# hip-satomi/microbeSEG

Measured on AMD Instinct MI355X. Metric: training crops/sec (256px), higher is better.
Workload: dtype f32; 1 GPU; BASELINE configs[1]: DU-Net distance-map training step, filters [64, 1024], 256x256 crops, per-GPU batch 32, fp32, relu/bn, SmoothL1x2 + Adam(amsgrad); global_batch=32, parallelism=dp1, launch=eager

## Files before the change

include/mseg_hip.h:

```cpp
#ifndef MSEG_HIP_H
#define MSEG_HIP_H

#include <stddef.h>
#include <stdint.h>

#ifdef __cplusplus
extern "C" {
#endif

#define MSEG_OK 0
#define MSEG_EINVAL (-1)
#define MSEG_ELAUNCH (-2)
#define MSEG_EWORKSPACE (-3)

#define MSEG_ACT_NONE 0
#define MSEG_ACT_RELU 1
#define MSEG_ACT_LEAKY 2
#define MSEG_ACT_ELU 3
#define MSEG_ACT_MISH 4

#define MSEG_NORM_BN 0
#define MSEG_NORM_GN 1
#define MSEG_NORM_IN 2

// ... 35 lines not shown
  float* stats;
  int32_t stats_act;
  int32_t reserved0;
} MsegIgemm;

int mseg_igemm(const MsegIgemm* p, void* stream);

typedef struct MsegKernelInfo {
  char name[120];
  int32_t precision;
  int32_t launches;
  uint32_t grid, block;
  size_t workspace;
  int32_t stats_rows;
  int32_t reserved0;
} MsegKernelInfo;
int mseg_igemm_query(const MsegIgemm* p, MsegKernelInfo* info);
const char* mseg_last_kernel(void);
int mseg_f32_to_bf16(const float* src, uint16_t* dst, size_t n, void* stream);
size_t mseg_igemm_workspace_bytes(const MsegIgemm* p);
int mseg_igemm_set_persistent(int on);
int mseg_igemm_set_wide_tiles(int on);
int mseg_igemm_set_p8(int mode);

typedef struct MsegWgrad {
  MsegSrc P;
  MsegSrc Q[2];
  float* ws;
  float* dst;
  int32_t nq, Nch, Nch_store;
  int32_t NB, Hp, Wp, Hq, Wq;
  int32_t KH, KW, stride, pad;
  int32_t splits;
  int32_t phase;
  int32_t precision;
  int32_t reserved;
} MsegWgrad;

size_t mseg_wgrad_workspace_bytes(const MsegWgrad* p);
int mseg_wgrad(const MsegWgrad* p, void* stream);
int mseg_wgrad_query(const MsegWgrad* p, MsegKernelInfo* info);

int mseg_first_conv_fwd(const float* x4, const float* w, const float* bias, int N, int H, int W, int Cin, int Cout,
                        void* z, int z_dtype, void* stream);
#define MSEG_PIX_U8 0
#define MSEG_PIX_U16 1
// ... 167 lines not shown
```

microbeseg_amd/_lib.py:

```python
import ctypes as C
import os
import pathlib

_HERE = pathlib.Path(__file__).resolve().parent
LIB_PATH = _HERE / "libmseg_hip.so"

ACT = {"none": 0, "relu": 1, "leakyrelu": 2, "elu": 3, "mish": 4}
NORM = {"bn": 0, "gn": 1, "in": 2}
MODE_CONV, MODE_TCONV = 0, 1
EPI_PLAIN, EPI_SCATTER2X2 = 0, 1
MORDER_LINEAR, MORDER_PARITY = 0, 1
ST_F32, ST_BF16 = 0, 1


class MsegLibraryError(RuntimeError):
    pass


class MsegSrc(C.Structure):
    _fields_ = [("ptr", C.c_void_p), ("scale", C.c_void_p), ("shift", C.c_void_p),
                ("C", C.c_int32), ("act", C.c_int32), ("ss", C.c_int32), ("dtype", C.c_int32)]


class MsegIgemm(C.Structure):
# ... 29 lines not shown
                ("first_block", C.c_uint32), ("reserved", C.c_uint32)]


class MsegRangerJob(C.Structure):
    _fields_ = [("p", C.c_void_p), ("g", C.c_void_p), ("m", C.c_void_p), ("v", C.c_void_p), ("slow", C.c_void_p),
                ("n", C.c_uint64), ("rows", C.c_int32), ("step_lr", C.c_float), ("flags", C.c_uint32),
                ("reserved", C.c_uint32)]


_P = C.c_void_p
_I = C.c_int
_F = C.c_float
_D = C.c_double
_SZ = C.c_size_t

SIGNATURES = {
    "mseg_igemm": (_I, [C.POINTER(MsegIgemm), _P]),
    "mseg_igemm_workspace_bytes": (_SZ, [C.POINTER(MsegIgemm)]),
    "mseg_igemm_query": (_I, [C.POINTER(MsegIgemm), C.POINTER(MsegKernelInfo)]),
    "mseg_last_kernel": (C.c_char_p, []),
    "mseg_igemm_set_persistent": (_I, [_I]),
    "mseg_igemm_set_wide_tiles": (_I, [_I]),
    "mseg_igemm_set_p8": (_I, [_I]),
    "mseg_f32_to_bf16": (_I, [_P, _P, _SZ, _P]),
    "mseg_first_conv_fwd": (_I, [_P, _P, _P, _I, _I, _I, _I, _I, _P, _I, _P]),
    "mseg_frame_minmax": (_I, [_P, _I, _SZ, _P, _P]),
    "mseg_first_conv_fwd_raw": (_I, [_P, _I, _I, _I, _I, _I, _P, _P, _P, _I, _P, _I, _P]),
    "mseg_frame_normalize": (_I, [_P, _I, _I, _I, _I, _I, _P, _P, _P]),
    "mseg_first_wgrad_workspace_bytes": (_SZ, [_I, _I, _I, _I]),
    "mseg_first_wgrad": (_I, [_P, _P, _I, _I, _I, _I, _I, _P, _P, _P]),
    "mseg_wgrad_workspace_bytes": (_SZ, [C.POINTER(MsegWgrad)]),
    "mseg_wgrad": (_I, [C.POINTER(MsegWgrad), _P]),
    "mseg_wgrad_query": (_I, [C.POINTER(MsegWgrad), C.POINTER(MsegKernelInfo)]),
    "mseg_pack_weight": (_I, [_P, _P, _I, _I, _I, _I, _I, _I, _I, _I, _P]),
    "mseg_pack_job_blocks": (C.c_uint, [_I, _I, _I]),
    "mseg_pack_weights_multi": (_I, [_P, _I, C.c_uint, _P]),
    "mseg_norm_workspace_bytes": (_SZ, [_I, _I, _I]),
    "mseg_norm_set_tails": (_I, [_I]),
    "mseg_norm_set_finish": (_I, [_I]),
    "mseg_norm_stats_from_conv": (_I, [_P, _I, _I, C.c_longlong, _P, _P, _F, _P, _P, _P, _P, _P, _P, _F, _P, _P]),
    "mseg_norm_stats": (_I, [_P, _I, _I, _I, _I, _I, _I, _P, _P, _F, _P, _P, _P, _P, _P, _P, _F, _P, _P, _P]),
    "mseg_activation": (_I, [_P, _I, _I, _I, _I, _I, _P, _P]),
    "mseg_bn_eval_coeffs": (_I, [_P, _P, _P, _P, _F, _I, _P, _P, _P]),
    "mseg_norm_bwd": (_I, [_P, _P, _I, _I, _I, _I, _I, _I, _P, _P, _P, _P, _P, _P, _P, _P, _P, _P]),
    "mseg_maxpool2x2_fwd": (_I, [C.POINTER(MsegSrc), _I, _I, _I, _P, _P]),
    "mseg_maxpool2x2_bwd": (_I, [C.POINTER(MsegSrc), _I, _I, _I, _P, _P, _I, _P]),
# ... 95 lines not shown
```

microbeseg_amd/csrc/igemm.hip:

```cpp
#include "common.h"
#include "igemm_common.h"
#include "bf16_affine.h"

int igemm_p8_try(const MsegIgemm& p, int tr, int m_fastest, int cus, hipStream_t st);

__device__ float g_ident_scale[MSEG_MAX_CH];
__device__ float g_ident_shift[MSEG_MAX_CH];
__global__ void init_ident_kernel() {
  for (int i = blockIdx.x * blockDim.x + threadIdx.x; i < MSEG_MAX_CH; i += gridDim.x * blockDim.x) {
    g_ident_scale[i] = 1.f;
    g_ident_shift[i] = 0.f;
  }
}


template <int BM, int BN, bool PER_SAMPLE, bool GENERIC_ACT>
__global__ __launch_bounds__(256) void igemm_kernel(const MsegIgemm p) {
  using Cfg = IgemmCfg<BM, BN>;
  constexpr int STAGE = (BM + BN) * LDS_STRIDE;
  __shared__ __attribute__((aligned(16))) float lds[2 * STAGE + 4];
  unsigned* tapmask_s = reinterpret_cast<unsigned*>(lds + 2 * STAGE);

  const int tid = threadIdx.x;
  const int lane = tid & 63;
  const int wave = tid >> 6;
  const int wm = wave / Cfg::WN, wn = wave % Cfg::WN;

// ... 186 lines not shown
    }
    float* An = lds + (cur ^ 1) * STAGE;
#ifdef MSEG_ABLATE
    STAMP(s2);
    if (!(abl & 8)) commit(An, An + BM * LDS_STRIDE);
    STAMP(s3);
    if (!(abl & 2)) __syncthreads();
    STAMP(s4);
    t_issue += s1 - s0; t_mfma += s2 - s1; t_commit += s3 - s2; t_bar += s4 - s3;
#else
    commit(An, An + BM * LDS_STRIDE);
    __syncthreads();
#endif
    cur ^= 1;
    have = have_next;
  }

#ifdef MSEG_ABLATE
  if ((abl & 32) && p.dst1 && lane == 0 && blockIdx.x < 1024) {
    float* dbg = p.dst1 + ((size_t)blockIdx.x * 4 + wave) * 4;
    dbg[0] = (float)t_issue; dbg[1] = (float)t_mfma; dbg[2] = (float)t_commit; dbg[3] = (float)t_bar;
  }
#endif
  igemm_epilogue<IgemmCfg<BM, BN>>(acc, m0, n0, wm, wn, lane, M);
}

template <int BM, int BN, int TR, bool PER_SAMPLE, bool SB = false>
__global__ __launch_bounds__(256) void igemm_fast_kernel(const MsegIgemm p) {
  using Cfg = IgemmCfg<BM, BN>;
  constexpr int STAGE = (BM + BN) * LDS_STRIDE;
  __shared__ __attribute__((aligned(16))) float lds[(SB ? 1 : 2) * STAGE];

  const int tid = threadIdx.x;
  const int lane = tid & 63;
  const int wave = tid >> 6;
  const int wm = wave / Cfg::WN, wn = wave % Cfg::WN;
  const int M = p.NB * p.Ho * p.Wo;
  const int ntiles_n = (p.Ngemm + BN - 1) / BN;
  const int lid = (int)xcd_logical_id(blockIdx.x, gridDim.x);
  const int tile_m = lid / ntiles_n;
  const int tile_n = lid - tile_m * ntiles_n;
  const int m0 = tile_m * BM, n0 = tile_n * BN;
  const int T = p.KH * p.KW;
  const int srow = tid >> 3, scol = tid & 7;

  const TapGeom geom = make_geom(p);
  const long long tile_px = tile_base_pixel(p, geom, m0, M);
  int pix0[Cfg::AROWS];
  int rown[Cfg::AROWS];
  unsigned vmask[Cfg::AROWS];
#pragma unroll
  for (int i = 0; i < Cfg::AROWS; ++i) {
    const RowInfo r = decode_row(p, m0 + srow + 32 * i, M);
    const int iy0 = (r.oy * geom.sm - geom.dir * geom.pad) >> geom.sh, ix0 = (r.ox * geom.sm - geom.dir * geom.pad) >> geom.sh;
    pix0[i] = (int)(((long long)r.n * p.Hi + iy0) * p.Wi + ix0 - tile_px);
    rown[i] = r.n < 0 ? 0 : r.n;
    unsigned mk = 0u;
    for (int t = 0; t < T; ++t) {
      const int ky = t / p.KW, kx = t - ky * p.KW;
      int iy, ix;
      mk |= (unsigned)tap_coord(geom, r, ky, kx, iy, ix) << t;
    }
    vmask[i] = mk;
  }

  f32x16 acc[Cfg::MB][Cfg::NB];
#pragma unroll
  for (int a = 0; a < Cfg::MB; ++a)
#pragma unroll
    for (int b = 0; b < Cfg::NB; ++b)
#pragma unroll
      for (int r = 0; r < 16; ++r) acc[a][b][r] = 0.f;

  const int nchunks = (p.Cin + KC - 1) / KC;
  const int C0 = p.src[0].C;
  const unsigned OOB = 0x80000000u;

  const __amdgpu_buffer_rsrc_t rs0 = __builtin_amdgcn_make_buffer_rsrc(
      const_cast<float*>(p.src[0].ptr + tile_px * p.src[0].C), 0, 0x7ffffff0, 0x00020000);
  const __amdgpu_buffer_rsrc_t rs1 = __builtin_amdgcn_make_buffer_rsrc(
      const_cast<float*>((p.nsrc > 1 ? p.src[1].ptr : p.src[0].ptr) + tile_px * (p.nsrc > 1 ? p.src[1].C : p.src[0].C)), 0,
      0x7ffffff0, 0x00020000);
  const __amdgpu_buffer_rsrc_t rsw = __builtin_amdgcn_make_buffer_rsrc(const_cast<float*>(p.w), 0,
                                                                        T * p.Npad * p.Kpad * 4, 0x00020000);
  unsigned wvoff[Cfg::BROWS];
#pragma unroll
  for (int i = 0; i < Cfg::BROWS; ++i) wvoff[i] = ((unsigned)(n0 + srow + 32 * i) * (unsigned)p.Kpad + scol * 4u) * 4u;

  constexpr int NSC = (TR == 0) ? 1 : (PER_SAMPLE ? Cfg::AROWS : 1);
  float4 ra[Cfg::AROWS], rb[Cfg::BROWS], rsc[NSC], rsh[NSC];
  float rm[Cfg::AROWS];
  unsigned rowoff[Cfg::AROWS];
  int ract = 0;
  int cur_chunk = -1;
  bool cur_s1 = false;

  auto issue = [&](int chunk, int t, int ky, int kx) {
    const int c = chunk * KC + scol * 4;
    if (chunk != cur_chunk) {
      cur_chunk = chunk;
      cur_s1 = (p.nsrc > 1) && (chunk * KC >= C0);
      const unsigned sC4 = (unsigned)(cur_s1 ? p.src[1].C : p.src[0].C) * 4u;
      const unsigned cl4 = (unsigned)(cur_s1 ? c - C0 : c) * 4u;
#pragma unroll
      for (int i = 0; i < Cfg::AROWS; ++i) rowoff[i] = (unsigned)pix0[i] * sC4 + cl4;
      if (TR != 0) {
        const MsegSrc& s = cur_s1 ? p.src[1] : p.src[0];
        ract = s.act;
        const bool has_aff = s.scale != nullptr;
        const float* scp = has_aff ? s.scale : g_ident_scale;
        const float* shp = has_aff ? s.shift : g_ident_shift;
        const unsigned cl = (c < p.Cin) ? (cl4 >> 2) : 0u;
#pragma unroll
        for (int i = 0; i < NSC; ++i) {
          const size_t o = (size_t)(PER_SAMPLE ? rown[i] : 0) * (has_aff ? (unsigned)s.ss : 0u) + cl;
          rsc[i] = *reinterpret_cast<const float4*>(scp + o);
          rsh[i] = *reinterpret_cast<const float4*>(shp + o);
        }
      }
    }
    const unsigned cbit = (c < p.Cin) ? (1u << t) : 0u;
    const unsigned sC4 = (unsigned)(cur_s1 ? p.src[1].C : p.src[0].C) * 4u;
    const unsigned delta = (unsigned)(geom.dir * ((ky >> geom.sh) * p.Wi + (kx >> geom.sh))) * sC4;
#pragma unroll
    for (int i = 0; i < Cfg::AROWS; ++i) {
      const bool ok = (vmask[i] & cbit) != 0u;
      const unsigned vo = ok ? rowoff[i] + delta : OOB;
      const f32x4 v = cur_s1 ? __builtin_bit_cast(f32x4, __builtin_amdgcn_raw_buffer_load_b128(rs1, vo, 0, 0))
                             : __builtin_bit_cast(f32x4, __builtin_amdgcn_raw_buffer_load_b128(rs0, vo, 0, 0));
      ra[i] = make_float4(v[0], v[1], v[2], v[3]);
      if (TR != 0) rm[i] = ok ? 1.f : 0.f;
    }
    const unsigned wso = ((unsigned)t * (unsigned)p.Npad * (unsigned)p.Kpad + (unsigned)chunk * KC) * 4u;
#pragma unroll
    for (int i = 0; i < Cfg::BROWS; ++i) {
      const f32x4 v = __builtin_bit_cast(f32x4, __builtin_amdgcn_raw_buffer_load_b128(rsw, wvoff[i], wso, 0));
      rb[i] = make_float4(v[0], v[1], v[2], v[3]);
    }
  };

  auto commit = [&](float* As, float* Bs) {
    const float lo = (ract == MSEG_ACT_RELU) ? 0.f : -3.402823466e38f;
#pragma unroll
    for (int i = 0; i < Cfg::AROWS; ++i) {
      float4 v = ra[i];
      if (TR != 0) {
        if (TR == 2) {
          v = act_fwd4(v, ract);
        } else {
          v.x = clamp_lo(v.x, lo); v.y = clamp_lo(v.y, lo); v.z = clamp_lo(v.z, lo); v.w = clamp_lo(v.w, lo);
        }
        const float4 sc = rsc[PER_SAMPLE ? i : 0], sh = rsh[PER_SAMPLE ? i : 0];
        const float m = rm[i];
        v.x = (v.x * sc.x + sh.x) * m; v.y = (v.y * sc.y + sh.y) * m;
        v.z = (v.z * sc.z + sh.z) * m; v.w = (v.w * sc.w + sh.w) * m;
      }
      *reinterpret_cast<float4*>(As + (srow + 32 * i) * LDS_STRIDE + scol * 4) = v;
    }
#pragma unroll
    for (int i = 0; i < Cfg::BROWS; ++i)
      *reinterpret_cast<float4*>(Bs + (srow + 32 * i) * LDS_STRIDE + scol * 4) = rb[i];
  };

  unsigned long long taplist = 0ull, taplist_hi = 0ull;
  int nlive = 0;
  {
    int py = 0, px = 0;
    if (geom.sh) {
      const int cls = m0 / (M >> 2);
      py = cls >> 1; px = cls & 1;
    }
    for (int tt = 0; tt < T; ++tt) {
      const int ky_ = tt / p.KW, kx_ = tt - ky_ * p.KW;
      const bool live = (((py - geom.dir * (ky_ - geom.pad)) | (px - geom.dir * (kx_ - geom.pad))) & geom.sh) == 0;
      if (live) {
        const unsigned long long e = (unsigned long long)(tt | (ky_ << 4) | (kx_ << 6));
        if (nlive < 8) taplist |= e << (8 * nlive); else taplist_hi |= e << (8 * (nlive - 8));
        ++nlive;
      }
    }
  }
  auto tap_at = [&](int j) -> unsigned { return (unsigned)((j < 8 ? taplist >> (8 * j) : taplist_hi >> (8 * (j - 8))) & 0xffull); };
  int chunk = 0, j = 0;
  const int nsteps = nchunks * nlive;
  unsigned e0 = tap_at(0);
  issue(0, (int)(e0 & 15u), (int)((e0 >> 4) & 3u), (int)(e0 >> 6));
  commit(lds, lds + BM * LDS_STRIDE);
  __syncthreads();
  int cur = 0;
  const int li = lane & 31, lh = lane >> 5;
  for (int step = 0; step < nsteps; ++step) {
    if (step + 1 < nsteps) {
      j += 1;
      if (j >= nlive) { j = 0; ++chunk; }
    }
    e0 = tap_at(j);
    issue(chunk, (int)(e0 & 15u), (int)((e0 >> 4) & 3u), (int)(e0 >> 6));

    const float* As = lds + cur * STAGE;
    const float* Bs = As + BM * LDS_STRIDE;
#pragma unroll
    for (int kk = 0; kk < KC / 8; ++kk) {
      float4 af[Cfg::MB], bf[Cfg::NB];
#pragma unroll
      for (int a = 0; a < Cfg::MB; ++a)
        af[a] = *reinterpret_cast<const float4*>(As + (wm * Cfg::TM + a * 32 + li) * LDS_STRIDE + kk * 8 + lh * 4);
#pragma unroll
      for (int b = 0; b < Cfg::NB; ++b)
        bf[b] = *reinterpret_cast<const float4*>(Bs + (wn * Cfg::TN + b * 32 + li) * LDS_STRIDE + kk * 8 + lh * 4);
#pragma unroll
      for (int a = 0; a < Cfg::MB; ++a)
#pragma unroll
        for (int b = 0; b < Cfg::NB; ++b) {
          acc[a][b] = __builtin_amdgcn_mfma_f32_32x32x2f32(af[a].x, bf[b].x, acc[a][b], 0, 0, 0);
          acc[a][b] = __builtin_amdgcn_mfma_f32_32x32x2f32(af[a].y, bf[b].y, acc[a][b], 0, 0, 0);
          acc[a][b] = __builtin_amdgcn_mfma_f32_32x32x2f32(af[a].z, bf[b].z, acc[a][b], 0, 0, 0);
          acc[a][b] = __builtin_amdgcn_mfma_f32_32x32x2f32(af[a].w, bf[b].w, acc[a][b], 0, 0, 0);
        }
    }
    if (SB) {
      __syncthreads();
      commit(lds, lds + BM * LDS_STRIDE);
      __syncthreads();
    } else {
      float* An = lds + (cur ^ 1) * STAGE;
      commit(An, An + BM * LDS_STRIDE);
      __syncthreads();
      cur ^= 1;
    }
  }
  igemm_epilogue<IgemmCfg<BM, BN>>(acc, m0, n0, wm, wn, lane, M);
}

template <int BN>
struct HaloCfg {
  static constexpr int WN = (BN >= 128) ? 4 : 2;
  static constexpr int WM = 8 / WN;
  static constexpr int TM = 128 / WM, TN = BN / WN;
  static constexpr int MB = TM / 32, NB = TN / 32;
  static constexpr int BROWS = BN / 64;
};

template <int BN, int TR>
__global__ __launch_bounds__(512, 2) void igemm_halo_kernel(const MsegIgemm p, int tw_log2, int ksplit,
                                                            int chunks_per_split) {
  constexpr int BM = 128;
  using Cfg = HaloCfg<BN>;
  constexpr int HMAX = 264;
  constexpr int HL = (HMAX * 8 + 511) / 512;
  constexpr int ASTAGE = HMAX * LDS_STRIDE;
  constexpr int BSTAGE = BN * LDS_STRIDE;
  __shared__ __attribute__((aligned(16))) float lds[ASTAGE + 2 * BSTAGE];
  float* const Abuf = lds;
// ... 2183 lines not shown
    if (!fast) return MSEG_EINVAL;
    const int tr = plain ? 0 : (generic ? 2 : 1);
#define MSEG_FAST16_LAUNCH(BM_, BN_, TR_, PS_)                                                          \
  do {                                                                                                  \
    if (s16) MSEG_KL((igemm_fast_bf16_kernel<BM_, BN_, TR_, PS_, true>), grid, block, 0, st, p);   \
    else MSEG_KL((igemm_fast_bf16_kernel<BM_, BN_, TR_, PS_, false>), grid, block, 0, st, p);      \
  } while (0)
#define MSEG_FAST16_TILE(BM_, BN_)                                                        \
  do {                                                                                    \
    if (tr == 0) MSEG_FAST16_LAUNCH(BM_, BN_, 0, false);                                  \
    else if (tr == 1) { if (per_sample) MSEG_FAST16_LAUNCH(BM_, BN_, 1, true); else MSEG_FAST16_LAUNCH(BM_, BN_, 1, false); } \
    else { if (per_sample) MSEG_FAST16_LAUNCH(BM_, BN_, 2, true); else MSEG_FAST16_LAUNCH(BM_, BN_, 2, false); }              \
  } while (0)
    if (wide) MSEG_FAST16_TILE(128, 128); else MSEG_FAST16_TILE(128, 64);
#undef MSEG_FAST16_TILE
#undef MSEG_FAST16_LAUNCH
    MSEG_LAUNCH_CHECK();
    return MSEG_OK;
  }
  if (fast) {
    const int tr = plain ? 0 : (generic ? 2 : 1);
    const int live_taps = (p.mode == MSEG_MODE_TCONV && p.stride == 2) ? ((p.KH + 1) / 2) * ((p.KW + 1) / 2) : p.KH * p.KW;
    const bool short_k = ((p.Cin + KC - 1) / KC) * live_taps <= 8;
#define MSEG_FAST_LAUNCH(BM_, BN_, TR_, PS_)                                                              \
  do {                                                                                                    \
    if (short_k) MSEG_KL((igemm_fast_kernel<BM_, BN_, TR_, PS_, true>), grid, block, 0, st, p); \
    else MSEG_KL((igemm_fast_kernel<BM_, BN_, TR_, PS_, false>), grid, block, 0, st, p);        \
  } while (0)
#define MSEG_FAST_TILE(BM_, BN_)                                                          \
  do {                                                                                    \
    if (tr == 0) MSEG_FAST_LAUNCH(BM_, BN_, 0, false);                                    \
    else if (tr == 1) { if (per_sample) MSEG_FAST_LAUNCH(BM_, BN_, 1, true); else MSEG_FAST_LAUNCH(BM_, BN_, 1, false); } \
    else { if (per_sample) MSEG_FAST_LAUNCH(BM_, BN_, 2, true); else MSEG_FAST_LAUNCH(BM_, BN_, 2, false); }              \
  } while (0)
    if (wide) MSEG_FAST_TILE(128, 128); else MSEG_FAST_TILE(128, 64);
#undef MSEG_FAST_TILE
#undef MSEG_FAST_LAUNCH
    MSEG_LAUNCH_CHECK();
    return MSEG_OK;
  }
#define MSEG_IGEMM_LAUNCH(BM_, BN_, PS_, GA_) \
  MSEG_KL((igemm_kernel<BM_, BN_, PS_, GA_>), grid, block, 0, st, p)
  if (wide) {
    if (per_sample) { if (generic) MSEG_IGEMM_LAUNCH(128, 128, true, true); else MSEG_IGEMM_LAUNCH(128, 128, true, false); }
    else            { if (generic) MSEG_IGEMM_LAUNCH(128, 128, false, true); else MSEG_IGEMM_LAUNCH(128, 128, false, false); }
  } else {
    if (per_sample) { if (generic) MSEG_IGEMM_LAUNCH(128, 64, true, true); else MSEG_IGEMM_LAUNCH(128, 64, true, false); }
    else            { if (generic) MSEG_IGEMM_LAUNCH(128, 64, false, true); else MSEG_IGEMM_LAUNCH(128, 64, false, false); }
  }
#undef MSEG_IGEMM_LAUNCH
  MSEG_LAUNCH_CHECK();
  return MSEG_OK;
}

extern "C" int mseg_igemm(const MsegIgemm* pp, void* stream) {
  mseg_dispatch_begin(0);
  const int rc = igemm_dispatch(pp, stream);
  mseg_dispatch_end(nullptr);
  return rc;
}

extern "C" int mseg_igemm_query(const MsegIgemm* pp, MsegKernelInfo* info) {
// ... 98 lines not shown
```

microbeseg_amd/csrc/igemm_common.h:

```cpp
#pragma once
#include "common.h"

#define KC 32
#define LDS_STRIDE 36
#define MSEG_MAX_CH 8192

template <int BM, int BN>
struct IgemmCfg {
  static constexpr int WM = (BN >= 128) ? 2 : 4;
  static constexpr int WN = 4 / WM;
  static constexpr int TM = BM / WM;
  static constexpr int TN = BN / WN;
  static constexpr int MB = TM / 32;
  static constexpr int NB = TN / 32;
  static constexpr int AROWS = BM / 32;
  static constexpr int BROWS = BN / 32;
};

struct RowInfo {
  int n;
  int oy, ox;
};

__device__ __forceinline__ RowInfo decode_row(const MsegIgemm& p, int m, int M) {
// ... 182 lines not shown
      };
      if (mode == 0) { emit(rel_affine); continue; }
      if (mode == 1) { emit(rel_narrow); continue; }
      if (mode != 4) { emit(rel_walk); continue; }
#pragma unroll
      for (int r = 0; r < 16; ++r) {
        const int m = mb + (r & 3) + 8 * (r >> 2) + 4 * lh;
        if (m >= M) continue;
        const RowInfo ri = decode_row(*pe, m, M);
        const size_t off = (((size_t)ri.n * e_Ho + ri.oy) * e_Wo + ri.ox) * ld + noff;
        float v = acc[a][b][r] + bias;
        if (e_d16) {
          __bf16* const d = reinterpret_cast<__bf16*>(dst);
          if (accf) v += (float)d[off];
          d[off] = (__bf16)v;
        } else {
          if (accf) v += dst[off];
          dst[off] = v;
        }
      }
    }
  }
}
```

microbeseg_amd/engine.py:

```python
import ctypes as C
import os

import torch

from . import _lib
from ._lib import (ACT, NORM, MODE_CONV, MODE_TCONV, EPI_PLAIN, EPI_SCATTER2X2, MORDER_LINEAR, MORDER_PARITY,
                   ST_F32, ST_BF16, MsegSrc, MsegIgemm, MsegWgrad, MsegKernelInfo, check)

BN_EPS = 1e-5
BN_MOMENTUM = 0.1


def _ptr(t):
    return None if t is None else t.data_ptr()


def _stream():
    return torch.cuda.current_stream().cuda_stream


def _pad4(c):
    return (c + 3) // 4 * 4


# ... 372 lines not shown


_bf16_ok_cache = {}


def _igemm_bf16_ok(p):
    key = (p.nsrc, tuple((p.src[i].C, p.src[i].act, bool(p.src[i].scale), p.src[i].ss != 0, p.src[i].dtype)
                         for i in range(p.nsrc)), p.Kpad, p.Npad, p.NB, p.Hi, p.Wi, p.Ho, p.Wo, p.KH, p.KW, p.stride, p.pad,
           p.mode, p.morder, p.Ngemm, p.epi, p.split, p.ld0, p.ld1, p.acc0, p.acc1, p.Cq, p.dst_dtype, bool(p.bias))
    ok = _bf16_ok_cache.get(key)
    if ok is None:
        p.precision = 1
        ok = _bf16_ok_cache[key] = _query(_lib.load().mseg_igemm_query, p) is not None
    return ok


_conv_stats = os.environ.get("MSEG_CONV_STATS", "0") == "1"


def set_conv_stats(flag):
    global _conv_stats
    old, _conv_stats = _conv_stats, bool(flag)
    return old


def igemm(srcs, w, bias, NB, Hi, Wi, Ho, Wo, KH, KW, stride, pad, mode, Ngemm, dst0, ld0, acc0=0,
          dst1=None, ld1=0, acc1=0, split=None, epi=EPI_PLAIN, Cq=0, morder=MORDER_LINEAR, real_cin=None,
          precision=None, stats=None):
    lib = _lib.load()
    p = MsegIgemm()
    _fill_igemm(p, srcs, w.Kpad, w.Npad, NB, Hi, Wi, Ho, Wo, KH, KW, stride, pad, mode, Ngemm, ld0, acc0, ld1, acc1, split, epi,
                Cq, morder)
    p.w = w.t.data_ptr()
    p.dst_dtype = _st(dst0)
    p.bias = _ptr(bias)
    p.dst0 = dst0.data_ptr()
    p.dst1 = _ptr(dst1)
    bf16 = (precision or _precision) == "bf16" and _igemm_bf16_ok(p)
    if bf16:
        p.w = w.bf16().data_ptr()
    p.precision = 1 if bf16 else 0
    need = lib.mseg_igemm_workspace_bytes(C.byref(p))
    if need:
        key = (dst0.device, _stream())
        buf = _splitk_ws.get(key)
        if buf is None or buf.numel() < need:
# ... 653 lines not shown
```

Measured before the change: 245.3 crops/s.

## Add transposed-MFMA fast igemm variant with vectorized epilogue for stride-2 convs

```diff
diff --git a/include/mseg_hip.h b/include/mseg_hip.h
--- a/include/mseg_hip.h
+++ b/include/mseg_hip.h
@@ -81,6 +81,7 @@
 int mseg_igemm_set_persistent(int on);
 int mseg_igemm_set_wide_tiles(int on);
 int mseg_igemm_set_p8(int mode);
+int mseg_igemm_set_s2_forms(int on);
 
 typedef struct MsegWgrad {
   MsegSrc P;
diff --git a/microbeseg_amd/_lib.py b/microbeseg_amd/_lib.py
--- a/microbeseg_amd/_lib.py
+++ b/microbeseg_amd/_lib.py
@@ -75,6 +75,7 @@
     "mseg_igemm_set_persistent": (_I, [_I]),
     "mseg_igemm_set_wide_tiles": (_I, [_I]),
     "mseg_igemm_set_p8": (_I, [_I]),
+    "mseg_igemm_set_s2_forms": (_I, [_I]),
     "mseg_f32_to_bf16": (_I, [_P, _P, _SZ, _P]),
     "mseg_first_conv_fwd": (_I, [_P, _P, _P, _I, _I, _I, _I, _I, _P, _I, _P]),
     "mseg_frame_minmax": (_I, [_P, _I, _SZ, _P, _P]),
diff --git a/microbeseg_amd/csrc/igemm.hip b/microbeseg_amd/csrc/igemm.hip
--- a/microbeseg_amd/csrc/igemm.hip
+++ b/microbeseg_amd/csrc/igemm.hip
@@ -3,6 +3,7 @@
 #include "bf16_affine.h"
 
 int igemm_p8_try(const MsegIgemm& p, int tr, int m_fastest, int cus, hipStream_t st);
+int igemm_fast_launch(const MsegIgemm& p, int tr, bool per_sample, bool short_k, bool wide, dim3 grid, hipStream_t st);
 
 __device__ float g_ident_scale[MSEG_MAX_CH];
 __device__ float g_ident_shift[MSEG_MAX_CH];
@@ -235,213 +236,6 @@
     dbg[0] = (float)t_issue; dbg[1] = (float)t_mfma; dbg[2] = (float)t_commit; dbg[3] = (float)t_bar;
   }
 #endif
-  igemm_epilogue<IgemmCfg<BM, BN>>(acc, m0, n0, wm, wn, lane, M);
-}
-
-template <int BM, int BN, int TR, bool PER_SAMPLE, bool SB = false>
-__global__ __launch_bounds__(256) void igemm_fast_kernel(const MsegIgemm p) {
-  using Cfg = IgemmCfg<BM, BN>;
-  constexpr int STAGE = (BM + BN) * LDS_STRIDE;
-  __shared__ __attribute__((aligned(16))) float lds[(SB ? 1 : 2) * STAGE];
-
-  const int tid = threadIdx.x;
-  const int lane = tid & 63;
-  const int wave = tid >> 6;
-  const int wm = wave / Cfg::WN, wn = wave % Cfg::WN;
-  const int M = p.NB * p.Ho * p.Wo;
-  const int ntiles_n = (p.Ngemm + BN - 1) / BN;
-  const int lid = (int)xcd_logical_id(blockIdx.x, gridDim.x);
-  const int tile_m = lid / ntiles_n;
-  const int tile_n = lid - tile_m * ntiles_n;
-  const int m0 = tile_m * BM, n0 = tile_n * BN;
-  const int T = p.KH * p.KW;
-  const int srow = tid >> 3, scol = tid & 7;
-
-  const TapGeom geom = make_geom(p);
-  const long long tile_px = tile_base_pixel(p, geom, m0, M);
-  int pix0[Cfg::AROWS];
-  int rown[Cfg::AROWS];
-  unsigned vmask[Cfg::AROWS];
-#pragma unroll
-  for (int i = 0; i < Cfg::AROWS; ++i) {
-    const RowInfo r = decode_row(p, m0 + srow + 32 * i, M);
-    const int iy0 = (r.oy * geom.sm - geom.dir * geom.pad) >> geom.sh, ix0 = (r.ox * geom.sm - geom.dir * geom.pad) >> geom.sh;
-    pix0[i] = (int)(((long long)r.n * p.Hi + iy0) * p.Wi + ix0 - tile_px);
-    rown[i] = r.n < 0 ? 0 : r.n;
-    unsigned mk = 0u;
-    for (int t = 0; t < T; ++t) {
-      const int ky = t / p.KW, kx = t - ky * p.KW;
-      int iy, ix;
-      mk |= (unsigned)tap_coord(geom, r, ky, kx, iy, ix) << t;
-    }
-    vmask[i] = mk;
-  }
-
-  f32x16 acc[Cfg::MB][Cfg::NB];
-#pragma unroll
-  for (int a = 0; a < Cfg::MB; ++a)
-#pragma unroll
-    for (int b = 0; b < Cfg::NB; ++b)
-#pragma unroll
-      for (int r = 0; r < 16; ++r) acc[a][b][r] = 0.f;
-
-  const int nchunks = (p.Cin + KC - 1) / KC;
-  const int C0 = p.src[0].C;
-  const unsigned OOB = 0x80000000u;
-
-  const __amdgpu_buffer_rsrc_t rs0 = __builtin_amdgcn_make_buffer_rsrc(
-      const_cast<float*>(p.src[0].ptr + tile_px * p.src[0].C), 0, 0x7ffffff0, 0x00020000);
-  const __amdgpu_buffer_rsrc_t rs1 = __builtin_amdgcn_make_buffer_rsrc(
-      const_cast<float*>((p.nsrc > 1 ? p.src[1].ptr : p.src[0].ptr) + tile_px * (p.nsrc > 1 ? p.src[1].C : p.src[0].C)), 0,
-      0x7ffffff0, 0x00020000);
-  const __amdgpu_buffer_rsrc_t rsw = __builtin_amdgcn_make_buffer_rsrc(const_cast<float*>(p.w), 0,
-                                                                        T * p.Npad * p.Kpad * 4, 0x00020000);
-  unsigned wvoff[Cfg::BROWS];
-#pragma unroll
-  for (int i = 0; i < Cfg::BROWS; ++i) wvoff[i] = ((unsigned)(n0 + srow + 32 * i) * (unsigned)p.Kpad + scol * 4u) * 4u;
-
-  constexpr int NSC = (TR == 0) ? 1 : (PER_SAMPLE ? Cfg::AROWS : 1);
-  float4 ra[Cfg::AROWS], rb[Cfg::BROWS], rsc[NSC], rsh[NSC];
-  float rm[Cfg::AROWS];
-  unsigned rowoff[Cfg::AROWS];
-  int ract = 0;
-  int cur_chunk = -1;
-  bool cur_s1 = false;
-
-  auto issue = [&](int chunk, int t, int ky, int kx) {
-    const int c = chunk * KC + scol * 4;
-    if (chunk != cur_chunk) {
-      cur_chunk = chunk;
-      cur_s1 = (p.nsrc > 1) && (chunk * KC >= C0);
-      const unsigned sC4 = (unsigned)(cur_s1 ? p.src[1].C : p.src[0].C) * 4u;
-      const unsigned cl4 = (unsigned)(cur_s1 ? c - C0 : c) * 4u;
-#pragma unroll
-      for (int i = 0; i < Cfg::AROWS; ++i) rowoff[i] = (unsigned)pix0[i] * sC4 + cl4;
-      if (TR != 0) {
-        const MsegSrc& s = cur_s1 ? p.src[1] : p.src[0];
-        ract = s.act;
-        const bool has_aff = s.scale != nullptr;
-        const float* scp = has_aff ? s.scale : g_ident_scale;
-        const float* shp = has_aff ? s.shift : g_ident_shift;
-        const unsigned cl = (c < p.Cin) ? (cl4 >> 2) : 0u;
-#pragma unroll
-        for (int i = 0; i < NSC; ++i) {
-          const size_t o = (size_t)(PER_SAMPLE ? rown[i] : 0) * (has_aff ? (unsigned)s.ss : 0u) + cl;
-          rsc[i] = *reinterpret_cast<const float4*>(scp + o);
-          rsh[i] = *reinterpret_cast<const float4*>(shp + o);
-        }
-      }
-    }
-    const unsigned cbit = (c < p.Cin) ? (1u << t) : 0u;
-    const unsigned sC4 = (unsigned)(cur_s1 ? p.src[1].C : p.src[0].C) * 4u;
-    const unsigned delta = (unsigned)(geom.dir * ((ky >> geom.sh) * p.Wi + (kx >> geom.sh))) * sC4;
-#pragma unroll
-    for (int i = 0; i < Cfg::AROWS; ++i) {
-      const bool ok = (vmask[i] & cbit) != 0u;
-      const unsigned vo = ok ? rowoff[i] + delta : OOB;
-      const f32x4 v = cur_s1 ? __builtin_bit_cast(f32x4, __builtin_amdgcn_raw_buffer_load_b128(rs1, vo, 0, 0))
-                             : __builtin_bit_cast(f32x4, __builtin_amdgcn_raw_buffer_load_b128(rs0, vo, 0, 0));
-      ra[i] = make_float4(v[0], v[1], v[2], v[3]);
-      if (TR != 0) rm[i] = ok ? 1.f : 0.f;
-    }
-    const unsigned wso = ((unsigned)t * (unsigned)p.Npad * (unsigned)p.Kpad + (unsigned)chunk * KC) * 4u;
-#pragma unroll
-    for (int i = 0; i < Cfg::BROWS; ++i) {
-      const f32x4 v = __builtin_bit_cast(f32x4, __builtin_amdgcn_raw_buffer_load_b128(rsw, wvoff[i], wso, 0));
-      rb[i] = make_float4(v[0], v[1], v[2], v[3]);
-    }
-  };
-
-  auto commit = [&](float* As, float* Bs) {
-    const float lo = (ract == MSEG_ACT_RELU) ? 0.f : -3.402823466e38f;
-#pragma unroll
-    for (int i = 0; i < Cfg::AROWS; ++i) {
-      float4 v = ra[i];
-      if (TR != 0) {
-        if (TR == 2) {
-          v = act_fwd4(v, ract);
-        } else {
-          v.x = clamp_lo(v.x, lo); v.y = clamp_lo(v.y, lo); v.z = clamp_lo(v.z, lo); v.w = clamp_lo(v.w, lo);
-        }
-        const float4 sc = rsc[PER_SAMPLE ? i : 0], sh = rsh[PER_SAMPLE ? i : 0];
-        const float m = rm[i];
-        v.x = (v.x * sc.x + sh.x) * m; v.y = (v.y * sc.y + sh.y) * m;
-        v.z = (v.z * sc.z + sh.z) * m; v.w = (v.w * sc.w + sh.w) * m;
-      }
-      *reinterpret_cast<float4*>(As + (srow + 32 * i) * LDS_STRIDE + scol * 4) = v;
-    }
-#pragma unroll
-    for (int i = 0; i < Cfg::BROWS; ++i)
-      *reinterpret_cast<float4*>(Bs + (srow + 32 * i) * LDS_STRIDE + scol * 4) = rb[i];
-  };
-
-  unsigned long long taplist = 0ull, taplist_hi = 0ull;
-  int nlive = 0;
-  {
-    int py = 0, px = 0;
-    if (geom.sh) {
-      const int cls = m0 / (M >> 2);
-      py = cls >> 1; px = cls & 1;
-    }
-    for (int tt = 0; tt < T; ++tt) {
-      const int ky_ = tt / p.KW, kx_ = tt - ky_ * p.KW;
-      const bool live = (((py - geom.dir * (ky_ - geom.pad)) | (px - geom.dir * (kx_ - geom.pad))) & geom.sh) == 0;
-      if (live) {
-        const unsigned long long e = (unsigned long long)(tt | (ky_ << 4) | (kx_ << 6));
-        if (nlive < 8) taplist |= e << (8 * nlive); else taplist_hi |= e << (8 * (nlive - 8));
-        ++nlive;
-      }
-    }
-  }
-  auto tap_at = [&](int j) -> unsigned { return (unsigned)((j < 8 ? taplist >> (8 * j) : taplist_hi >> (8 * (j - 8))) & 0xffull); };
-  int chunk = 0, j = 0;
-  const int nsteps = nchunks * nlive;
-  unsigned e0 = tap_at(0);
-  issue(0, (int)(e0 & 15u), (int)((e0 >> 4) & 3u), (int)(e0 >> 6));
-  commit(lds, lds + BM * LDS_STRIDE);
-  __syncthreads();
-  int cur = 0;
-  const int li = lane & 31, lh = lane >> 5;
-  for (int step = 0; step < nsteps; ++step) {
-    if (step + 1 < nsteps) {
-      j += 1;
-      if (j >= nlive) { j = 0; ++chunk; }
-    }
-    e0 = tap_at(j);
-    issue(chunk, (int)(e0 & 15u), (int)((e0 >> 4) & 3u), (int)(e0 >> 6));
-
-    const float* As = lds + cur * STAGE;
-    const float* Bs = As + BM * LDS_STRIDE;
-#pragma unroll
-    for (int kk = 0; kk < KC / 8; ++kk) {
-      float4 af[Cfg::MB], bf[Cfg::NB];
-#pragma unroll
-      for (int a = 0; a < Cfg::MB; ++a)
-        af[a] = *reinterpret_cast<const float4*>(As + (wm * Cfg::TM + a * 32 + li) * LDS_STRIDE + kk * 8 + lh * 4);
-#pragma unroll
-      for (int b = 0; b < Cfg::NB; ++b)
-        bf[b] = *reinterpret_cast<const float4*>(Bs + (wn * Cfg::TN + b * 32 + li) * LDS_STRIDE + kk * 8 + lh * 4);
-#pragma unroll
-      for (int a = 0; a < Cfg::MB; ++a)
-#pragma unroll
-        for (int b = 0; b < Cfg::NB; ++b) {
-          acc[a][b] = __builtin_amdgcn_mfma_f32_32x32x2f32(af[a].x, bf[b].x, acc[a][b], 0, 0, 0);
-          acc[a][b] = __builtin_amdgcn_mfma_f32_32x32x2f32(af[a].y, bf[b].y, acc[a][b], 0, 0, 0);
-          acc[a][b] = __builtin_amdgcn_mfma_f32_32x32x2f32(af[a].z, bf[b].z, acc[a][b], 0, 0, 0);
-          acc[a][b] = __builtin_amdgcn_mfma_f32_32x32x2f32(af[a].w, bf[b].w, acc[a][b], 0, 0, 0);
-        }
-    }
-    if (SB) {
-      __syncthreads();
-      commit(lds, lds + BM * LDS_STRIDE);
-      __syncthreads();
-    } else {
-      float* An = lds + (cur ^ 1) * STAGE;
-      commit(An, An + BM * LDS_STRIDE);
-      __syncthreads();
-      cur ^= 1;
-    }
-  }
   igemm_epilogue<IgemmCfg<BM, BN>>(acc, m0, n0, wm, wn, lane, M);
 }
 
@@ -2671,22 +2465,7 @@
     const int tr = plain ? 0 : (generic ? 2 : 1);
     const int live_taps = (p.mode == MSEG_MODE_TCONV && p.stride == 2) ? ((p.KH + 1) / 2) * ((p.KW + 1) / 2) : p.KH * p.KW;
     const bool short_k = ((p.Cin + KC - 1) / KC) * live_taps <= 8;
-#define MSEG_FAST_LAUNCH(BM_, BN_, TR_, PS_)                                                              \
-  do {                                                                                                    \
-    if (short_k) MSEG_KL((igemm_fast_kernel<BM_, BN_, TR_, PS_, true>), grid, block, 0, st, p); \
-    else MSEG_KL((igemm_fast_kernel<BM_, BN_, TR_, PS_, false>), grid, block, 0, st, p);        \
-  } while (0)
-#define MSEG_FAST_TILE(BM_, BN_)                                                          \
-  do {                                                                                    \
-    if (tr == 0) MSEG_FAST_LAUNCH(BM_, BN_, 0, false);                                    \
-    else if (tr == 1) { if (per_sample) MSEG_FAST_LAUNCH(BM_, BN_, 1, true); else MSEG_FAST_LAUNCH(BM_, BN_, 1, false); } \
-    else { if (per_sample) MSEG_FAST_LAUNCH(BM_, BN_, 2, true); else MSEG_FAST_LAUNCH(BM_, BN_, 2, false); }              \
-  } while (0)
-    if (wide) MSEG_FAST_TILE(128, 128); else MSEG_FAST_TILE(128, 64);
-#undef MSEG_FAST_TILE
-#undef MSEG_FAST_LAUNCH
-    MSEG_LAUNCH_CHECK();
-    return MSEG_OK;
+    return igemm_fast_launch(p, tr, per_sample, short_k, wide, grid, st);
   }
 #define MSEG_IGEMM_LAUNCH(BM_, BN_, PS_, GA_) \
   MSEG_KL((igemm_kernel<BM_, BN_, PS_, GA_>), grid, block, 0, st, p)
diff --git a/microbeseg_amd/csrc/igemm_common.h b/microbeseg_amd/csrc/igemm_common.h
--- a/microbeseg_amd/csrc/igemm_common.h
+++ b/microbeseg_amd/csrc/igemm_common.h
@@ -228,3 +228,95 @@
     }
   }
 }
+
+template <typename Cfg, typename AccT>
+__device__ __forceinline__ void igemm_epilogue_x4(AccT& acc , int m0, int n0, int wm, int wn,
+                                                  int lane, int M) {
+  const int li = lane & 31, lh = lane >> 5;
+  const MsegIgemm* pe = (const MsegIgemm*)__builtin_amdgcn_kernarg_segment_ptr();
+  asm volatile("" : "+s"(pe));
+  const float* e_bias = pe->bias;
+  float* e_dst0 = pe->dst0;
+  float* e_dst1 = pe->dst1;
+  const int e_epi = pe->epi, e_split = pe->split, e_ld0 = pe->ld0, e_ld1 = pe->ld1, e_acc0 = pe->acc0,
+            e_acc1 = pe->acc1, e_Cq = pe->Cq, e_morder = pe->morder, e_Ho = pe->Ho, e_Wo = pe->Wo, e_Ngemm = pe->Ngemm;
+  const bool scatter = e_epi == MSEG_EPI_SCATTER2X2;
+  const int nw = n0 + wn * Cfg::TN;
+  const int ab_w = scatter ? nw / e_Cq : 0;
+  const int co_w = nw - ab_w * e_Cq;
+#pragma unroll
+  for (int a = 0; a < Cfg::MB; ++a) {
+    const int mb = m0 + wm * Cfg::TM + a * 32;
+    if (mb >= M) continue;
+    const int rows_left = M - mb;
+    size_t pbase;
+    unsigned relpix;
+    if (scatter || e_morder == MSEG_MORDER_PARITY) {
+      const int Wg = scatter ? e_Wo : (e_Wo >> 1), Hg = scatter ? e_Ho : (e_Ho >> 1);
+      const int Wd = scatter ? 2 * e_Wo : e_Wo, Hd = scatter ? 2 * e_Ho : e_Ho;
+      int cls = 0, rem = mb;
+      if (!scatter) {
+        const int per = M >> 2;
+        cls = mb / per;
+        rem = mb - cls * per;
+      }
+      const int b_img = rem / (Hg * Wg);
+      const int r2 = rem - b_img * (Hg * Wg);
+      const int b_y = r2 / Wg, b_x = r2 - b_y * Wg;
+      pbase = ((size_t)b_img * Hd + 2 * b_y + (cls >> 1)) * Wd + 2 * b_x + (cls & 1);
+      int x = b_x + li, y = b_y, img = b_img;
+      while (x >= Wg) { x -= Wg; ++y; }
+      while (y >= Hg) { y -= Hg; ++img; }
+      relpix = (unsigned)((((img - b_img) * Hd + 2 * (y - b_y)) * Wd) + 2 * (x - b_x));
+    } else {
+      pbase = (size_t)mb;
+      relpix = (unsigned)li;
+    }
+    const bool rvalid = li < rows_left;
+    int ab = ab_w, co = co_w;
+#pragma unroll
+    for (int b = 0; b < Cfg::NB; ++b) {
+      float* dq[4];
+      unsigned off[4];
+      const float* bq[4];
+      bool live[4], accq[4];
+#pragma unroll
+      for (int q = 0; q < 4; ++q) {
+        const int nq = nw + b * 32 + 8 * q;
+        live[q] = nq < e_Ngemm;
+        float* dst = e_dst0;
+        int ld = e_ld0, noff = nq, accf = e_acc0;
+        size_t padd = 0;
+        if (scatter) {
+          padd = (size_t)(ab >> 1) * (2 * e_Wo) + (ab & 1);
+          ld = e_Cq; noff = co;
+          co += 8;
+          if (co >= e_Cq) { co -= e_Cq; ++ab; }
+        } else if (nq >= e_split) {
+          dst = e_dst1; ld = e_ld1; noff = nq - e_split; accf = e_acc1;
+        }
+        dq[q] = dst + ((pbase + padd) * (size_t)ld + noff);
+        off[q] = relpix * (unsigned)ld + 4u * lh;
+        bq[q] = e_bias ? e_bias + (scatter ? noff : nq) : nullptr;
+        accq[q] = accf != 0;
+      }
+      float4 old[4], bias[4];
+#pragma unroll
+      for (int q = 0; q < 4; ++q) {
+        old[q] = make_float4(0.f, 0.f, 0.f, 0.f);
+        bias[q] = make_float4(0.f, 0.f, 0.f, 0.f);
+        if (live[q] && bq[q]) bias[q] = *reinterpret_cast<const float4*>(bq[q] + 4 * lh);
+        if (live[q] && accq[q] && rvalid) old[q] = *reinterpret_cast<const float4*>(dq[q] + off[q]);
+      }
+#pragma unroll
+      for (int q = 0; q < 4; ++q) {
+        float4 v;
+        v.x = acc[a][b][4 * q + 0] + bias[q].x + old[q].x;
+        v.y = acc[a][b][4 * q + 1] + bias[q].y + old[q].y;
+        v.z = acc[a][b][4 * q + 2] + bias[q].z + old[q].z;
+        v.w = acc[a][b][4 * q + 3] + bias[q].w + old[q].w;
+        if (live[q] && rvalid) *reinterpret_cast<float4*>(dq[q] + off[q]) = v;
+      }
+    }
+  }
+}
diff --git a/microbeseg_amd/csrc/igemm_fast.hip b/microbeseg_amd/csrc/igemm_fast.hip
--- /dev/null
+++ b/microbeseg_amd/csrc/igemm_fast.hip
@@ -0,0 +1,301 @@
+#include "common.h"
+#include "igemm_common.h"
+#include <stdlib.h>
+
+__device__ float g_ident_scale[MSEG_MAX_CH];
+__device__ float g_ident_shift[MSEG_MAX_CH];
+__global__ void init_fast_ident_kernel() {
+  for (int i = blockIdx.x * blockDim.x + threadIdx.x; i < MSEG_MAX_CH; i += gridDim.x * blockDim.x) {
+    g_ident_scale[i] = 1.f;
+    g_ident_shift[i] = 0.f;
+  }
+}
+
+template <int BM, int BN, int TR, bool PER_SAMPLE, bool SB = false, int X4 = 0>
+__global__ __launch_bounds__(256, (SB && X4) ? (BN == 128 ? 3 : 4) : 1) void igemm_fast_kernel(const MsegIgemm p) {
+  using Cfg = IgemmCfg<BM, BN>;
+  constexpr int STAGE = (BM + BN) * LDS_STRIDE;
+  __shared__ __attribute__((aligned(16))) float lds[(SB ? 1 : 2) * STAGE];
+
+  const int tid = threadIdx.x;
+  const int lane = tid & 63;
+  const int wave = tid >> 6;
+  const int wm = wave / Cfg::WN, wn = wave % Cfg::WN;
+  const int M = p.NB * p.Ho * p.Wo;
+  const int ntiles_n = (p.Ngemm + BN - 1) / BN;
+  const int lid = (int)xcd_logical_id(blockIdx.x, gridDim.x);
+  int tile_m = lid / ntiles_n;
+  const int tile_n = lid - tile_m * ntiles_n;
+  if (X4 && p.morder == MSEG_MORDER_PARITY) {
+    const int per_class = (M >> 2) / BM;
+    tile_m = (tile_m & 3) * per_class + (tile_m >> 2);
+  }
+  const int m0 = tile_m * BM, n0 = tile_n * BN;
+  const int T = p.KH * p.KW;
+  const int srow = tid >> 3, scol = tid & 7;
+
+  const TapGeom geom = make_geom(p);
+  const long long tile_px = tile_base_pixel(p, geom, m0, M);
+  int pix0[Cfg::AROWS];
+  int rown[Cfg::AROWS];
+  unsigned vmask[Cfg::AROWS];
+#pragma unroll
+  for (int i = 0; i < Cfg::AROWS; ++i) {
+    const RowInfo r = decode_row(p, m0 + srow + 32 * i, M);
+    const int iy0 = (r.oy * geom.sm - geom.dir * geom.pad) >> geom.sh, ix0 = (r.ox * geom.sm - geom.dir * geom.pad) >> geom.sh;
+    pix0[i] = (int)(((long long)r.n * p.Hi + iy0) * p.Wi + ix0 - tile_px);
+    rown[i] = r.n < 0 ? 0 : r.n;
+    unsigned mk = 0u;
+    for (int t = 0; t < T; ++t) {
+      const int ky = t / p.KW, kx = t - ky * p.KW;
+      int iy, ix;
+      mk |= (unsigned)tap_coord(geom, r, ky, kx, iy, ix) << t;
+    }
+    vmask[i] = mk;
+  }
+
+  f32x16 acc[Cfg::MB][Cfg::NB];
+#pragma unroll
+  for (int a = 0; a < Cfg::MB; ++a)
+#pragma unroll
+    for (int b = 0; b < Cfg::NB; ++b)
+#pragma unroll
+      for (int r = 0; r < 16; ++r) acc[a][b][r] = 0.f;
+
+  const int nchunks = (p.Cin + KC - 1) / KC;
+  const int C0 = p.src[0].C;
+  const unsigned OOB = 0x80000000u;
+
+  const __amdgpu_buffer_rsrc_t rs0 = __builtin_amdgcn_make_buffer_rsrc(
+      const_cast<float*>(p.src[0].ptr + tile_px * p.src[0].C), 0, 0x7ffffff0, 0x00020000);
+  const __amdgpu_buffer_rsrc_t rs1 = __builtin_amdgcn_make_buffer_rsrc(
+      const_cast<float*>((p.nsrc > 1 ? p.src[1].ptr : p.src[0].ptr) + tile_px * (p.nsrc > 1 ? p.src[1].C : p.src[0].C)), 0,
+      0x7ffffff0, 0x00020000);
+  const __amdgpu_buffer_rsrc_t rsw = __builtin_amdgcn_make_buffer_rsrc(const_cast<float*>(p.w), 0,
+                                                                        T * p.Npad * p.Kpad * 4, 0x00020000);
+  unsigned wvoff[Cfg::BROWS];
+#pragma unroll
+  for (int i = 0; i < Cfg::BROWS; ++i) wvoff[i] = ((unsigned)(n0 + srow + 32 * i) * (unsigned)p.Kpad + scol * 4u) * 4u;
+
+  constexpr int NSC = (TR == 0) ? 1 : (PER_SAMPLE ? Cfg::AROWS : 1);
+  float4 ra[Cfg::AROWS], rb[Cfg::BROWS], rsc[NSC], rsh[NSC];
+  float rm[Cfg::AROWS];
+  unsigned rowoff[Cfg::AROWS];
+  int ract = 0;
+  int cur_chunk = -1;
+  bool cur_s1 = false;
+
+  auto issue = [&](int chunk, int t, int ky, int kx) {
+    const int c = chunk * KC + scol * 4;
+    if (chunk != cur_chunk) {
+      cur_chunk = chunk;
+      cur_s1 = (p.nsrc > 1) && (chunk * KC >= C0);
+      const unsigned sC4 = (unsigned)(cur_s1 ? p.src[1].C : p.src[0].C) * 4u;
+      const unsigned cl4 = (unsigned)(cur_s1 ? c - C0 : c) * 4u;
+#pragma unroll
+      for (int i = 0; i < Cfg::AROWS; ++i) rowoff[i] = (unsigned)pix0[i] * sC4 + cl4;
+      if (TR != 0) {
+        const MsegSrc& s = cur_s1 ? p.src[1] : p.src[0];
+        ract = s.act;
+        const bool has_aff = s.scale != nullptr;
+        const float* scp = has_aff ? s.scale : g_ident_scale;
+        const float* shp = has_aff ? s.shift : g_ident_shift;
+        const unsigned cl = (c < p.Cin) ? (cl4 >> 2) : 0u;
+#pragma unroll
+        for (int i = 0; i < NSC; ++i) {
+          const size_t o = (size_t)(PER_SAMPLE ? rown[i] : 0) * (has_aff ? (unsigned)s.ss : 0u) + cl;
+          rsc[i] = *reinterpret_cast<const float4*>(scp + o);
+          rsh[i] = *reinterpret_cast<const float4*>(shp + o);
+        }
+      }
+    }
+    const unsigned cbit = (c < p.Cin) ? (1u << t) : 0u;
+    const unsigned sC4 = (unsigned)(cur_s1 ? p.src[1].C : p.src[0].C) * 4u;
+    const unsigned delta = (unsigned)(geom.dir * ((ky >> geom.sh) * p.Wi + (kx >> geom.sh))) * sC4;
+#pragma unroll
+    for (int i = 0; i < Cfg::AROWS; ++i) {
+      const bool ok = (vmask[i] & cbit) != 0u;
+      const unsigned vo = ok ? rowoff[i] + delta : OOB;
+      const f32x4 v = cur_s1 ? __builtin_bit_cast(f32x4, __builtin_amdgcn_raw_buffer_load_b128(rs1, vo, 0, 0))
+                             : __builtin_bit_cast(f32x4, __builtin_amdgcn_raw_buffer_load_b128(rs0, vo, 0, 0));
+      ra[i] = make_float4(v[0], v[1], v[2], v[3]);
+      if (TR != 0) rm[i] = ok ? 1.f : 0.f;
+    }
+    const unsigned wso = ((unsigned)t * (unsigned)p.Npad * (unsigned)p.Kpad + (unsigned)chunk * KC) * 4u;
+#pragma unroll
+    for (int i = 0; i < Cfg::BROWS; ++i) {
+      const f32x4 v = __builtin_bit_cast(f32x4, __builtin_amdgcn_raw_buffer_load_b128(rsw, wvoff[i], wso, 0));
+      rb[i] = make_float4(v[0], v[1], v[2], v[3]);
+    }
+  };
+
+  auto commit = [&](float* As, float* Bs) {
+    const float lo = (ract == MSEG_ACT_RELU) ? 0.f : -3.402823466e38f;
+#pragma unroll
+    for (int i = 0; i < Cfg::AROWS; ++i) {
+      float4 v = ra[i];
+      if (TR != 0) {
+        if (TR == 2) {
+          v = act_fwd4(v, ract);
+        } else {
+          v.x = clamp_lo(v.x, lo); v.y = clamp_lo(v.y, lo); v.z = clamp_lo(v.z, lo); v.w = clamp_lo(v.w, lo);
+        }
+        const float4 sc = rsc[PER_SAMPLE ? i : 0], sh = rsh[PER_SAMPLE ? i : 0];
+        const float m = rm[i];
+        v.x = (v.x * sc.x + sh.x) * m; v.y = (v.y * sc.y + sh.y) * m;
+        v.z = (v.z * sc.z + sh.z) * m; v.w = (v.w * sc.w + sh.w) * m;
+      }
+      *reinterpret_cast<float4*>(As + (srow + 32 * i) * LDS_STRIDE + scol * 4) = v;
+    }
+#pragma unroll
+    for (int i = 0; i < Cfg::BROWS; ++i)
+      *reinterpret_cast<float4*>(Bs + (srow + 32 * i) * LDS_STRIDE + scol * 4) = rb[i];
+  };
+
+  unsigned long long taplist = 0ull, taplist_hi = 0ull;
+  int nlive = 0;
+  {
+    int py = 0, px = 0;
+    if (geom.sh) {
+      const int cls = m0 / (M >> 2);
+      py = cls >> 1; px = cls & 1;
+    }
+    for (int tt = 0; tt < T; ++tt) {
+      const int ky_ = tt / p.KW, kx_ = tt - ky_ * p.KW;
+      const bool live = (((py - geom.dir * (ky_ - geom.pad)) | (px - geom.dir * (kx_ - geom.pad))) & geom.sh) == 0;
+      if (live) {
+        const unsigned long long e = (unsigned long long)(tt | (ky_ << 4) | (kx_ << 6));
+        if (nlive < 8) taplist |= e << (8 * nlive); else taplist_hi |= e << (8 * (nlive - 8));
+        ++nlive;
+      }
+    }
+  }
+  auto tap_at = [&](int j) -> unsigned { return (unsigned)((j < 8 ? taplist >> (8 * j) : taplist_hi >> (8 * (j - 8))) & 0xffull); };
+  int chunk = 0, j = 0;
+  const int nsteps = nchunks * nlive;
+  unsigned e0 = tap_at(0);
+  issue(0, (int)(e0 & 15u), (int)((e0 >> 4) & 3u), (int)(e0 >> 6));
+  commit(lds, lds + BM * LDS_STRIDE);
+  __syncthreads();
+  int cur = 0;
+  const int li = lane & 31, lh = lane >> 5;
+  for (int step = 0; step < nsteps; ++step) {
+    if (step + 1 < nsteps) {
+      j += 1;
+      if (j >= nlive) { j = 0; ++chunk; }
+    }
+    e0 = tap_at(j);
+    issue(chunk, (int)(e0 & 15u), (int)((e0 >> 4) & 3u), (int)(e0 >> 6));
+
+    const float* As = lds + cur * STAGE;
+    const float* Bs = As + BM * LDS_STRIDE;
+#pragma unroll
+    for (int kk = 0; kk < KC / 8; ++kk) {
+      float4 af[Cfg::MB], bf[Cfg::NB];
+#pragma unroll
+      for (int a = 0; a < Cfg::MB; ++a)
+        af[a] = *reinterpret_cast<const float4*>(As + (wm * Cfg::TM + a * 32 + li) * LDS_STRIDE + kk * 8 + lh * 4);
+#pragma unroll
+      for (int b = 0; b < Cfg::NB; ++b)
+        bf[b] = *reinterpret_cast<const float4*>(Bs + (wn * Cfg::TN + b * 32 + li) * LDS_STRIDE + kk * 8 + lh * 4);
+#pragma unroll
+      for (int a = 0; a < Cfg::MB; ++a)
+#pragma unroll
+        for (int b = 0; b < Cfg::NB; ++b) {
+          if (X4) {
+            acc[a][b] = __builtin_amdgcn_mfma_f32_32x32x2f32(bf[b].x, af[a].x, acc[a][b], 0, 0, 0);
+            acc[a][b] = __builtin_amdgcn_mfma_f32_32x32x2f32(bf[b].y, af[a].y, acc[a][b], 0, 0, 0);
+            acc[a][b] = __builtin_amdgcn_mfma_f32_32x32x2f32(bf[b].z, af[a].z, acc[a][b], 0, 0, 0);
+            acc[a][b] = __builtin_amdgcn_mfma_f32_32x32x2f32(bf[b].w, af[a].w, acc[a][b], 0, 0, 0);
+          } else {
+            acc[a][b] = __builtin_amdgcn_mfma_f32_32x32x2f32(af[a].x, bf[b].x, acc[a][b], 0, 0, 0);
+            acc[a][b] = __builtin_amdgcn_mfma_f32_32x32x2f32(af[a].y, bf[b].y, acc[a][b], 0, 0, 0);
+            acc[a][b] = __builtin_amdgcn_mfma_f32_32x32x2f32(af[a].z, bf[b].z, acc[a][b], 0, 0, 0);
+            acc[a][b] = __builtin_amdgcn_mfma_f32_32x32x2f32(af[a].w, bf[b].w, acc[a][b], 0, 0, 0);
+          }
+        }
+    }
+    if (SB) {
+      __syncthreads();
+      commit(lds, lds + BM * LDS_STRIDE);
+      __syncthreads();
+    } else {
+      float* An = lds + (cur ^ 1) * STAGE;
+      commit(An, An + BM * LDS_STRIDE);
+      __syncthreads();
+      cur ^= 1;
+    }
+  }
+  if (X4) igemm_epilogue_x4<IgemmCfg<BM, BN>>(acc, m0, n0, wm, wn, lane, M);
+  else igemm_epilogue<IgemmCfg<BM, BN>>(acc, m0, n0, wm, wn, lane, M);
+}
+
+static int g_s2_forms = -1;
+static int s2_forms_on() {
+  if (g_s2_forms < 0) {
+    const char* e = getenv("MSEG_S2_FORMS");
+    g_s2_forms = (e && e[0] == '0') ? 0 : 1;
+  }
+  return g_s2_forms;
+}
+extern "C" int mseg_igemm_set_s2_forms(int on) {
+  const int old = s2_forms_on();
+  g_s2_forms = on ? 1 : 0;
+  return old;
+}
+
+static bool x4_ok(const MsegIgemm& p) {
+  if (!s2_forms_on() || p.dst_dtype != MSEG_ST_F32) return false;
+  if (!(p.morder == MSEG_MORDER_PARITY || p.epi == MSEG_EPI_SCATTER2X2 ||
+        (p.mode == MSEG_MODE_CONV && p.stride == 2 && p.KH == 3 && p.KW == 3)))
+    return false;
+  const bool two = p.epi == MSEG_EPI_PLAIN && p.split < p.Ngemm;
+  if (p.Ngemm & 7) return false;
+  if (((uintptr_t)p.dst0 | (uintptr_t)p.bias) & 15) return false;
+  if (p.epi == MSEG_EPI_SCATTER2X2) return (p.Cq & 7) == 0 && (p.Wo & 15) == 0;
+  if ((p.ld0 & 3) || (two && ((p.split & 7) || (p.ld1 & 3) || ((uintptr_t)p.dst1 & 15)))) return false;
+  const int wg = p.morder == MSEG_MORDER_PARITY ? (p.Wo >> 1) : p.Wo;
+  return (wg & 15) == 0;
+}
+
+int igemm_fast_launch(const MsegIgemm& p, int tr, bool per_sample, bool short_k, bool wide, dim3 grid, hipStream_t st) {
+  const dim3 block(256);
+  static bool ident_ready[64] = {false};
+  if (!mseg_dispatch_dry()) {
+    int devid = 0;
+    if (hipGetDevice(&devid) != hipSuccess || devid < 0 || devid >= 64) return MSEG_ELAUNCH;
+    if (!ident_ready[devid]) {
+      MSEG_KL_AUX(init_fast_ident_kernel, dim3(8), dim3(256), 0, st);
+      MSEG_LAUNCH_CHECK();
+      ident_ready[devid] = true;
+    }
+  }
+  if (tr != 2 && !per_sample && x4_ok(p)) {
+#define MSEG_FAST_X4(BM_, BN_, TR_)                                                                   \
+  do {                                                                                                \
+    if (short_k) MSEG_KL((igemm_fast_kernel<BM_, BN_, TR_, false, true, 1>), grid, block, 0, st, p);  \
+    else MSEG_KL((igemm_fast_kernel<BM_, BN_, TR_, false, false, 1>), grid, block, 0, st, p);         \
+  } while (0)
+    if (wide) { if (tr == 0) MSEG_FAST_X4(128, 128, 0); else MSEG_FAST_X4(128, 128, 1); }
+    else      { if (tr == 0) MSEG_FAST_X4(128, 64, 0); else MSEG_FAST_X4(128, 64, 1); }
+#undef MSEG_FAST_X4
+    MSEG_LAUNCH_CHECK();
+    return MSEG_OK;
+  }
+#define MSEG_FAST_LAUNCH(BM_, BN_, TR_, PS_)                                                              \
+  do {                                                                                                    \
+    if (short_k) MSEG_KL((igemm_fast_kernel<BM_, BN_, TR_, PS_, true>), grid, block, 0, st, p); \
+    else MSEG_KL((igemm_fast_kernel<BM_, BN_, TR_, PS_, false>), grid, block, 0, st, p);        \
+  } while (0)
+#define MSEG_FAST_TILE(BM_, BN_)                                                          \
+  do {                                                                                    \
+    if (tr == 0) MSEG_FAST_LAUNCH(BM_, BN_, 0, false);                                    \
+    else if (tr == 1) { if (per_sample) MSEG_FAST_LAUNCH(BM_, BN_, 1, true); else MSEG_FAST_LAUNCH(BM_, BN_, 1, false); } \
+    else { if (per_sample) MSEG_FAST_LAUNCH(BM_, BN_, 2, true); else MSEG_FAST_LAUNCH(BM_, BN_, 2, false); }              \
+  } while (0)
+  if (wide) MSEG_FAST_TILE(128, 128); else MSEG_FAST_TILE(128, 64);
+#undef MSEG_FAST_TILE
+#undef MSEG_FAST_LAUNCH
+  MSEG_LAUNCH_CHECK();
+  return MSEG_OK;
+}
diff --git a/microbeseg_amd/engine.py b/microbeseg_amd/engine.py
--- a/microbeseg_amd/engine.py
+++ b/microbeseg_amd/engine.py
@@ -418,6 +418,10 @@
     global _conv_stats
     old, _conv_stats = _conv_stats, bool(flag)
     return old
+
+
+def set_s2_forms(flag):
+    return bool(_lib.load().mseg_igemm_set_s2_forms(1 if flag else 0))
 
 
 def igemm(srcs, w, bias, NB, Hi, Wi, Ho, Wo, KH, KW, stride, pad, mode, Ngemm, dst0, ld0, acc0=0,
```

Result: no change. 245.8 crops/s (median of 6 runs) (+0.2%).
